# Aman-4-Real/MMTG

Measured on AMD Instinct MI355X. Metric: train tokens/sec, full MMTG config (GPT-2-base-zh decoder, 5x(img+text) 2048-d WenLan embs), higher is better.
Workload: dtype bf16; 1 GPU; Full MMTG train step: S=5 experience steps, T=15+221=236 decoder positions, GPT-2 12L/768/12H V=13317, dropout 0.1 on, MyLoss stage 3 + 0.2*KL, clip 1.0, AdamW; rows_per_gpu=64, global_rows=64, seq_len=236, parallelism=single GPU, no collective

## Files before the change

### include/mmtg_hip.h

```cpp
#ifndef MMTG_HIP_H
#define MMTG_HIP_H

#ifdef __cplusplus
extern "C" {
#endif

#define MMTG_ABI_VERSION 12

#define MMTG_API __attribute__((visibility("default")))

enum { MMTG_OK = 0, MMTG_ERR_BAD_ARG = -1, MMTG_ERR_HIP = -2, MMTG_ERR_UNSUPPORTED = -3 };
enum { MMTG_F32 = 0, MMTG_BF16 = 1 };

enum {
    MMTG_EPI_NONE = 0,
    MMTG_EPI_GELU = 1,
    MMTG_EPI_TANH = 2,
    MMTG_EPI_RESID = 3,
    MMTG_EPI_DGELU = 4,
    MMTG_EPI_DTANH = 5,
    MMTG_EPI_ATOMIC = 6,
    MMTG_EPI_ROWDOT = 7,
    MMTG_EPI_SPLIT = 8,
    MMTG_EPI_TANH_ADD = 9
// ... 128 lines not shown
                      void* dgi, long ld_dgi, void* dgh, float* dh_prev, int B, int H, void* stream);
MMTG_API int mmtg_gru_cell_bwd_fused(int dtype, const void* rows, long ld_rows, const float* carry, const float* part, int splits,
                            const float* save, const void* h_prev, long ld_hp, void* dgi, long ld_dgi, void* dgh,
                            float* dh_prev, int B, int H, void* stream);
#define MMTG_RNN_RELU 0
#define MMTG_RNN_LSTM 1
MMTG_API int mmtg_rnn_cell_fwd(int dtype, int kind, const void* gi, long ld_gi, const void* gh, long ld_gh, const float* c_prev,
                      void* h, long ld_h, float* c, float* save, int B, int H, void* stream);
MMTG_API int mmtg_rnn_cell_bwd(int dtype, int kind, const void* rows, long ld_rows, const float* part, const float* save,
                      const float* c_prev, const void* h, long ld_h, float* dc, int dc_in, void* da, long ld_da,
                      int B, int H, void* stream);
MMTG_API int mmtg_alpha_attn_fwd(int dtype, const void* qkv, const float* prior, void* ctx, float* probs,
                        float* kl, int B, int S, int H, int heads, void* stream);
MMTG_API int mmtg_alpha_attn_bwd(int dtype, const void* qkv, const float* prior, const float* probs,
                        const void* dctx, float dkl, void* dqkv, int B, int S, int H, int heads,
                        void* stream);
MMTG_API int mmtg_beta_fuse_fwd(int dtype, const void* topic, const void* img, const void* txt,
                       const float* att_w, const float* att_b, void* o, float* a,
                       int B, int S, int H, void* stream);
MMTG_API long mmtg_beta_fuse_bwd_ws(int B, int S, int H);
MMTG_API int mmtg_beta_fuse_bwd(int dtype, const void* topic, const void* img, const void* txt,
                       const float* att_w, const float* a, const void* d_o,
                       float* dtopic, void* dimg, void* dtxt, float* datt_w, float* datt_b,
                       int B, int S, int H, float* ws, long ws_floats, void* stream);

MMTG_API int mmtg_prefetch(const void* src, long bytes, int workgroups, void* sink, void* stream);
MMTG_API int mmtg_zero_ranges(float* base, const long* desc, int n, void* stream);

MMTG_API long mmtg_sumsq_ws(long n);
MMTG_API int mmtg_sumsq(const float* x, long n, float* out, float* ws, long ws_floats, void* stream);
MMTG_API int mmtg_adamw(float* p, const float* g, float* m, float* v, void* p_bf16, void* p_lo, long n,
               float lr, float beta1, float beta2, float eps, float wd, int step,
               const float* normsq, float max_norm, float grad_scale, const float* count, void* stream);
MMTG_API int mmtg_cast_f32_to(int dtype, const float* src, void* dst, long n, void* stream);
MMTG_API int mmtg_cast_pad_rows(int dtype, const float* src, long lds_, void* dst, long ldd, int rows, int cols, void* stream);
MMTG_API int mmtg_cast_to_f32(int dtype, const void* src, float* dst, long n, void* stream);
MMTG_API int mmtg_axpy_f32(float* y, const float* x, float a, long n, void* stream);
MMTG_API int mmtg_slab_sum(const float* part, int splits, long stride, float* dst, int accumulate, long n, void* stream);
typedef struct mmtg_wgrad_problem {
    const void* A; long lda;
    const void* B; long ldb;
    float* C; long ldc;
    int M, N;
    long planeA, planeB;
} mmtg_wgrad_problem;
MMTG_API int mmtg_wgrad_group(int config, int n, const mmtg_wgrad_problem* probs, int K, int splits, float* ws, long ws_floats,
                     unsigned* counters, long n_counters, int accumulate, void* stream);
MMTG_API int mmtg_transpose_batch(int dtype, const void* src, void* dst, const long* desc, int n, int max_rows, int max_cols, void* stream);

MMTG_API int mmtg_logits_process_argmax(const float* logits, long ldl, int V, const long long* generated,
                               long ldg, const int* gen_len, float temperature, float rep_penalty,
                               long long* next, int B, void* stream);
MMTG_API int mmtg_logits_process_sample(const float* logits, long ldl, int V, const long long* generated, long ldg,
                               const int* gen_len, float temperature, float rep_penalty, int top_k, float top_p,
                               const float* uniforms, long long* next, float* filtered, int B, void* stream);

MMTG_API int mmtg_decode_embed(int dtype, const void* table, const long long* seq, long ldseq, const void* c, void* x,
                      const int* pos_ptr, const long long* tpw_type, const long long* tpw_mask,
                      long long* type_out, int* keep, long ldkeep, int B, int P, int S, int E, int two_sents,
                      int V, int sent, int max_sent_num, void* stream);
MMTG_API int mmtg_decode_embed_add(int dtype, const void* g, const void* wpe, const void* wte, const long long* type_ids,
                          const int* pos_ptr, void* h, int B, int D, float* stats, void* stream);
MMTG_API int mmtg_decode_gemm(int mode, int M, int N, int K, const void* A, long lda, const void* W, long ldw, void* C, long ldc,
                     const float* bias, const float* colsum, const float* stats_in, int np_in, float eps, int act, int out_f32,
                     const void* resid, long ldr, float* stats_out, int splits, float* ws, long ws_floats, unsigned* counters,
                     long n_counters, const void* emb_pos, const void* emb_type, const long long* type_ids, const int* pos_ptr,
// ... 133 lines not shown
```

### mmtg_amd/csrc/optim.hip

```cpp
#include "common.h"

namespace {

__global__ __launch_bounds__(256) void sumsq_kernel(const float* __restrict__ x, long n, float* __restrict__ out) {
    __shared__ float sh[4];
    float a = 0.f;
    const long n4 = n >> 2;
    for (long i = (long)blockIdx.x * 256 + threadIdx.x; i < n4; i += (long)gridDim.x * 256) {
        f32x4 v = reinterpret_cast<const f32x4*>(x)[i];
        a += v[0] * v[0] + v[1] * v[1] + v[2] * v[2] + v[3] * v[3];
    }
    if (blockIdx.x == 0)
        for (long i = (n4 << 2) + threadIdx.x; i < n; i += 256) a += x[i] * x[i];
    a = wave_sum(a);
    if ((threadIdx.x & 63) == 0) sh[threadIdx.x >> 6] = a;
    __syncthreads();
    if (threadIdx.x == 0) out[blockIdx.x] = sh[0] + sh[1] + sh[2] + sh[3];
}

__global__ __launch_bounds__(256) void sumsq_final_kernel(const float* __restrict__ part, int n, float* __restrict__ out) {
    __shared__ float sh[4];
    float a = 0.f;
    for (int i = threadIdx.x; i < n; i += 256) a += part[i];
    a = wave_sum(a);
// ... 22 lines not shown
    for (long i = (long)blockIdx.x * 256 + threadIdx.x; i < n4; i += (long)gridDim.x * 256) {
        const f32x4 g4 = reinterpret_cast<const f32x4*>(g)[i];
        f32x4 m4 = reinterpret_cast<f32x4*>(m)[i], v4 = reinterpret_cast<f32x4*>(v)[i], p4 = reinterpret_cast<f32x4*>(p)[i];
        bf16x4 c4, l4;
#pragma unroll
        for (int e = 0; e < 4; ++e) {
            const float gi = g4[e] * coef;
            const float mi = b1 * m4[e] + (1.f - b1) * gi;
            const float vi = b2 * v4[e] + (1.f - b2) * gi * gi;
            float pi = p4[e] - step_size * (mi / (sqrtf(vi) + eps));
            if (wd > 0.f) pi -= lr * wd * pi;
            m4[e] = mi; v4[e] = vi; p4[e] = pi;
            c4[e] = (bf16)pi;
            l4[e] = (bf16)(pi - (float)c4[e]);
        }
        reinterpret_cast<f32x4*>(m)[i] = m4;
        reinterpret_cast<f32x4*>(v)[i] = v4;
        reinterpret_cast<f32x4*>(p)[i] = p4;
        if (pc) reinterpret_cast<bf16x4*>(pc)[i] = c4;
        if (pl) reinterpret_cast<bf16x4*>(pl)[i] = l4;
    }
    for (long i = (n4 << 2) + (long)blockIdx.x * 256 + threadIdx.x; i < n; i += (long)gridDim.x * 256) {
        const float gi = g[i] * coef;
        const float mi = b1 * m[i] + (1.f - b1) * gi;
        const float vi = b2 * v[i] + (1.f - b2) * gi * gi;
        float pi = p[i] - step_size * (mi / (sqrtf(vi) + eps));
        if (wd > 0.f) pi -= lr * wd * pi;
        m[i] = mi; v[i] = vi; p[i] = pi;
        if (pc) pc[i] = (bf16)pi;
        if (pl) pl[i] = (bf16)(pi - (float)(bf16)pi);
    }
}

template <typename T>
__global__ __launch_bounds__(256) void cast_from_f32_kernel(const float* __restrict__ src, T* __restrict__ dst, long n) {
    for (long i = (long)blockIdx.x * 256 + threadIdx.x; i < n; i += (long)gridDim.x * 256) dst[i] = (T)src[i];
}
template <typename T>
__global__ __launch_bounds__(256) void cast_to_f32_kernel(const T* __restrict__ src, float* __restrict__ dst, long n) {
    for (long i = (long)blockIdx.x * 256 + threadIdx.x; i < n; i += (long)gridDim.x * 256) dst[i] = (float)src[i];
}
template <typename T>
__global__ __launch_bounds__(256) void cast_pad_rows_kernel(const float* __restrict__ src, long lds_, T* __restrict__ dst,
                                                            long ldd, int cols) {
    const long r = blockIdx.x;
    for (int c = threadIdx.x; c < ldd; c += 256) dst[r * ldd + c] = c < cols ? (T)src[r * lds_ + c] : (T)0.f;
}
__global__ __launch_bounds__(256) void axpy_kernel(float* __restrict__ y, const float* __restrict__ x, float a, long n) {
    for (long i = (long)blockIdx.x * 256 + threadIdx.x; i < n; i += (long)gridDim.x * 256) y[i] += a * x[i];
}

__global__ __launch_bounds__(256) void slab_sum_kernel(const float* __restrict__ part, int splits, long stride,
                                                       float* __restrict__ dst, int accumulate, long n4) {
    typedef float f4 __attribute__((ext_vector_type(4)));
    for (long i = (long)blockIdx.x * 256 + threadIdx.x; i < n4; i += (long)gridDim.x * 256) {
        const f4* src = reinterpret_cast<const f4*>(part) + i;
        f4 acc = accumulate ? reinterpret_cast<const f4*>(dst)[i] : f4{0.f, 0.f, 0.f, 0.f};
        int s = 0;
        for (; s + 4 <= splits; s += 4) {
            const f4 a = src[(s + 0) * (stride / 4)], b = src[(s + 1) * (stride / 4)];
            const f4 c = src[(s + 2) * (stride / 4)], d = src[(s + 3) * (stride / 4)];
            acc += a; acc += b; acc += c; acc += d;
        }
        for (; s < splits; ++s) acc += src[s * (stride / 4)];
        reinterpret_cast<f4*>(dst)[i] = acc;
    }
// ... 68 lines not shown
    MMTG_LAUNCH_CHECK("zero_ranges");
    return MMTG_OK;
}

extern "C" long mmtg_sumsq_ws(long n) { return (long)grid_for(n / 4 + 1); }

extern "C" int mmtg_sumsq(const float* x, long n, float* out, float* ws, long ws_floats, void* stream) {
    MMTG_REQUIRE(x && out && n > 0 && MMTG_ALIGNED16(x), "sumsq: bad args");
    const int g = grid_for(n / 4 + 1);
    MMTG_REQUIRE(ws && ws_floats >= g, "sumsq: workspace of %d floats required (mmtg_sumsq_ws)", g);
    hipStream_t s = (hipStream_t)stream;
    ProfScope prof(MMTG_PROF_OPTIM, s, 2.0 * n, 4.0 * n);
    hipLaunchKernelGGL(sumsq_kernel, dim3(g), dim3(256), 0, s, x, n, ws);
    hipLaunchKernelGGL(sumsq_final_kernel, dim3(1), dim3(256), 0, s, (const float*)ws, g, out);
    MMTG_LAUNCH_CHECK("sumsq");
    return MMTG_OK;
}

extern "C" int mmtg_adamw(float* p, const float* g, float* m, float* v, void* p_bf16, void* p_lo, long n,
                          float lr, float beta1, float beta2, float eps, float wd, int step,
                          const float* normsq, float max_norm, float grad_scale, const float* count, void* stream) {
    MMTG_REQUIRE(p && g && m && v && n > 0 && step >= 1, "adamw: bad args");
    MMTG_REQUIRE(!p_lo || p_bf16, "adamw: the lo plane comes with the hi plane (p_bf16)");
    hipStream_t s = (hipStream_t)stream;
    ProfScope prof(MMTG_PROF_OPTIM, s, 12.0 * n, (28.0 + (p_bf16 ? 2 : 0) + (p_lo ? 2 : 0)) * n);
    const double bc1 = 1.0 - pow((double)beta1, step), bc2 = 1.0 - pow((double)beta2, step);
    const float step_size = (float)((double)lr * sqrt(bc2) / bc1);
    hipLaunchKernelGGL(adamw_kernel, dim3(grid_for(n / 4 + 1)), dim3(256), 0, s, p, g, m, v, (bf16*)p_bf16, (bf16*)p_lo, n, lr, beta1, beta2,
                       eps, wd, step_size, normsq, max_norm, grad_scale, count);
    MMTG_LAUNCH_CHECK("adamw");
    return MMTG_OK;
}

extern "C" int mmtg_cast_f32_to(int dtype, const float* src, void* dst, long n, void* stream) {
    MMTG_REQUIRE(src && dst && n > 0, "cast_f32_to: bad args");
    hipStream_t s = (hipStream_t)stream;
    ProfScope prof(MMTG_PROF_MISC, s, 0, 6.0 * n);
    if (dtype == MMTG_BF16) hipLaunchKernelGGL(cast_from_f32_kernel<bf16>, dim3(grid_for(n)), dim3(256), 0, s, src, (bf16*)dst, n);
    else if (dtype == MMTG_F32) hipLaunchKernelGGL(cast_from_f32_kernel<float>, dim3(grid_for(n)), dim3(256), 0, s, src, (float*)dst, n);
    else MMTG_FAIL(MMTG_ERR_BAD_ARG, "cast_f32_to: bad dtype");
    MMTG_LAUNCH_CHECK("cast_f32_to");
    return MMTG_OK;
}

extern "C" int mmtg_cast_to_f32(int dtype, const void* src, float* dst, long n, void* stream) {
    MMTG_REQUIRE(src && dst && n > 0, "cast_to_f32: bad args");
    hipStream_t s = (hipStream_t)stream;
    ProfScope prof(MMTG_PROF_MISC, s, 0, 6.0 * n);
    if (dtype == MMTG_BF16) hipLaunchKernelGGL(cast_to_f32_kernel<bf16>, dim3(grid_for(n)), dim3(256), 0, s, (const bf16*)src, dst, n);
    else if (dtype == MMTG_F32) hipLaunchKernelGGL(cast_to_f32_kernel<float>, dim3(grid_for(n)), dim3(256), 0, s, (const float*)src, dst, n);
    else MMTG_FAIL(MMTG_ERR_BAD_ARG, "cast_to_f32: bad dtype");
    MMTG_LAUNCH_CHECK("cast_to_f32");
    return MMTG_OK;
}

extern "C" int mmtg_cast_pad_rows(int dtype, const float* src, long lds_, void* dst, long ldd, int rows, int cols, void* stream) {
    MMTG_REQUIRE(src && dst && rows > 0 && cols > 0 && ldd >= cols && lds_ >= cols, "cast_pad_rows: bad args");
    hipStream_t s = (hipStream_t)stream;
    ProfScope prof(MMTG_PROF_MISC, s, 0, 6.0 * rows * cols);
    if (dtype == MMTG_BF16) hipLaunchKernelGGL(cast_pad_rows_kernel<bf16>, dim3(rows), dim3(256), 0, s, src, lds_, (bf16*)dst, ldd, cols);
    else if (dtype == MMTG_F32) hipLaunchKernelGGL(cast_pad_rows_kernel<float>, dim3(rows), dim3(256), 0, s, src, lds_, (float*)dst, ldd, cols);
    else MMTG_FAIL(MMTG_ERR_BAD_ARG, "cast_pad_rows: bad dtype");
    MMTG_LAUNCH_CHECK("cast_pad_rows");
    return MMTG_OK;
}

// ... 36 lines not shown
```

### mmtg_amd/engine.py

```python
from __future__ import annotations

import contextlib
import math

import numpy as np
import torch

from . import hip
from .configs import rnn_param_shapes

ALIGN = 64


class ParamLayout:

    def __init__(self, model_cfgs, gpt2_cfg):
        S = model_cfgs["seq_len"]
        E = model_cfgs["topic"]["input_dim"]
        H = model_cfgs["topic"]["hidden_dim"]
        D = gpt2_cfg["n_embd"]
        V = gpt2_cfg["vocab_size"]
        NP = gpt2_cfg["n_positions"]
        L = gpt2_cfg["n_layer"]
        self.Vpad = (V + 127) // 128 * 128
# ... 119 lines not shown
def _dist_rank():
    import torch.distributed as dist
    return dist.get_rank() if dist.is_available() and dist.is_initialized() else int(_os.environ.get("RANK", "0"))


_NO_OCC4 = bool(_os.environ.get("MMTG_GEMM_NO_OCC4"))
_WG_NUM = float(_os.environ.get("MMTG_WGRAD_NUM", "760"))
_WG_CAP = int(_os.environ.get("MMTG_WGRAD_CAP", "12"))
_NO_FEW_ROWS = bool(_os.environ.get("MMTG_NO_FEW_ROWS"))
_WGRAD_SLAB = not _os.environ.get("MMTG_WGRAD_ATOMIC")
_NO_GATHER = bool(_os.environ.get("MMTG_NO_GATHER"))
_PREFETCH = int(_os.environ.get("MMTG_PREFETCH", "0"))


def _wgrad_splits(M, N, K, occ4=False, slots=512, t_iter=1.1, t_fixed=6.0):
    tiles = ((M + 127) // 128) * ((N + 127) // 128)
    if occ4 and not _NO_OCC4:
        smax = max(1, K // 256)
        s = round(_WG_NUM / tiles) if tiles < 512 else round(2520.0 / tiles)
        return int(max(1, min(smax, s, _WG_CAP)))
    best, best_t = 1, None
    for s in range(1, 33):
        if s > 1 and K // s < 256:
            break
        rounds = -(-tiles * s // slots)
        t = rounds * (K / (64.0 * s) * t_iter + t_fixed) + tiles * s * 65536 / 1.3e6
        if best_t is None or t < best_t * 0.97:
            best, best_t = s, t
    return best


_LAZY_ZERO = _os.environ.get("MMTG_FULL_ZERO_GRAD") is None
_WTE_T = _os.environ.get("MMTG_NO_WTE_T") is None
_P8T = _os.environ.get("MMTG_GEMM_P8T", "0") != "0"
_WGRAD_GROUP = _os.environ.get("MMTG_WGRAD_GROUP", "1") != "0"
_WGRAD_GROUP_SPLITS = int(_os.environ.get("MMTG_WGRAD_GROUP_SPLITS", "0"))
_GELU_GRAD = _os.environ.get("MMTG_GELU_GRAD", "0") != "0"
_DEFER_SUMS = _os.environ.get("MMTG_DEFER_SUMS", "1") != "0"
_WGRAD_TAIL = int(_os.environ.get("MMTG_WGRAD_TAIL", "8"))
_TAIL_FORK_EARLY = _os.environ.get("MMTG_WGRAD_TAIL_FORK", "loop") == "loop"
_LMHEAD_GROUP = _os.environ.get("MMTG_LMHEAD_GROUP", "1") != "0"
_LMHEAD_GROUP_SPLITS = int(_os.environ.get("MMTG_LMHEAD_GROUP_SPLITS", "0"))
_WGRAD_STREAM = _os.environ.get("MMTG_WGRAD_STREAM", "0") != "0"
_ENC_STREAMS = _os.environ.get("MMTG_ENC_STREAMS", "0") != "0"
_HYBRID_ENC_BF16 = _os.environ.get("MMTG_HYBRID_ENC_BF16", "1") != "0"
_X3_WG_CFG = 6 if _os.environ.get("MMTG_WGRAD_X3_COMBINED", "1") != "0" else 2
_WGRAD_GROUP_CFG = int(_os.environ.get("MMTG_WGRAD_GROUP_CFG", "0"))


def _group_splits(tiles, K, slots=1024):
    if _WGRAD_GROUP_SPLITS > 0:
        return _WGRAD_GROUP_SPLITS
    return int(max(1, min(slots // max(1, tiles), K // 1024, 16)))


def _group_splits_x3(tiles, K):
    if _X3_WG_CFG != 6:
        return _group_splits(tiles, K)
    if _WGRAD_GROUP_SPLITS > 0:
        return _WGRAD_GROUP_SPLITS
    s = 512 // max(1, tiles)
    if s == 0:
        s = 2048 // tiles
    return int(max(1, min(s, K // 1024, 16)))


# ... 153 lines not shown
            if off < pos:
                return
            if off > pos:
                comp.append((pos, off - pos))
            pos = off + n
        if pos < self.layout.total:
            comp.append((pos, self.layout.total - pos))
        if not ranges or any(o % 4 or c % 4 for o, c in comp):
            return
        self._ow_desc[key] = (torch.tensor(comp, dtype=torch.int64, device=self.dev), frozenset(ranges))

    def _init_transposed(self):
        self.wt = None
        self.wte_t = None
        self.wt_entries = {}
        if self.dtype == hip.F32 and not self.x3:
            return
        pre, desc, off = "decoder.gpt2.transformer.", [], 0
        for l in range(self.sh.L):
            for nm in ("attn.c_attn", "attn.c_proj", "mlp.c_fc", "mlp.c_proj"):
                key = "%sh.%d.%s.weight" % (pre, l, nm)
                soff, shape, n = self.layout.entries[key]
                assert soff % 8 == 0 and shape[0] % 8 == 0 and shape[1] % 8 == 0
                desc.append((soff, shape[0], shape[1], off))
                self.wt_entries[key] = (off, (shape[1], shape[0]), n)
                off += n
        if self.x3:
            key = "decoder.projector_layer2.weight"
            soff, shape, n = self.layout.entries[key]
            if soff % 8 == 0 and shape[0] % 8 == 0 and shape[1] % 8 == 0:
                desc.append((soff, shape[0], shape[1], off))
                self.wt_entries[key] = (off, (shape[1], shape[0]), n)
                off += n
        self.wt = torch.zeros(*((2, off) if self.x3 else (off,)), device=self.dev, dtype=torch.bfloat16)
        self.wt_total = off
        self.wt_desc = torch.tensor(desc, dtype=torch.int64, device=self.dev)
        self.wt_max = (max(d[1] for d in desc), max(d[2] for d in desc))
        woff = self.layout.pack_range["wte"][0]
        self.wte_t = (torch.zeros(*((2,) if self.x3 else ()), self.sh.D, self.layout.Vpad, device=self.dev, dtype=torch.bfloat16)
                      if (_WTE_T or self.x3) else None)
        self.wte_desc = torch.tensor([(woff, self.layout.Vpad, self.sh.D, 0)], dtype=torch.int64, device=self.dev)

    def Wt(self, key):
        if self.x3:
            raise RuntimeError("Engine.Wt: an x3 engine's transposed copies are (hi | lo) plane pairs -- use Wtx()")
        off, shape, n = self.wt_entries[key]
        return self.wt[off:off + n].view(shape)

    def _refresh_transposed(self):
        if self.wt is not None and self.x3:
            for pl in (0, 1):
                hip.transpose_batch(self.wc2[pl], self.wt[pl], self.wt_desc, self.wt_desc.shape[0], *self.wt_max)
                hip.transpose_batch(self.wc2[pl], self.wte_t[pl], self.wte_desc, 1, self.layout.Vpad, self.sh.D)
        elif self.wt is not None:
            hip.transpose_batch(self.wc, self.wt, self.wt_desc, self.wt_desc.shape[0], *self.wt_max)
            if self.wte_t is not None:
                hip.transpose_batch(self.wc, self.wte_t, self.wte_desc, 1, self.layout.Vpad, self.sh.D)

    def refresh_copies(self):
        if self.copies_fresh:
            return
        if self.x3:
            hip.split_planes(self.master, 1, self.layout.total, hip.Planes(self.wc2, 1, self.layout.total))
            self._refresh_transposed()
            self.copies_fresh = True
        elif self.dtype != hip.F32:
            hip.cast_f32_to(self.master, self.wc, self.layout.total)
            self._refresh_transposed()
            self.copies_fresh = True

    def invalidate_copies(self):
        if self.dtype != hip.F32 or self.x3:
            self.copies_fresh = False

# ... 971 lines not shown
                    last = t == S - 1
                    hip.rnn_cell_bwd(code, dh_all[t:], S * H, None if last else tmp32, save[t] if lstm else None,
                                     rec["c"][t - 1] if lstm and t else None, h_all[t:], S * H, dc, not last, dgi[t:], S * G * H, B, H)
                    if t > 0:
                        hip.gemm(dgi[t:], self.W(r + "weight_hh" + sfx), tmp32, B, H, G * H, transB=False, lda=S * G * H, ldb=H,
                                 out_f32=True)
                hip.colsum(dgi, B * S, G * H, self.G(r + "bias_hh" + sfx))
                drec_tm = None
                if S > 1:
                    drec_tm = self.buf("d_a_tm%d" % G, (S - 1, B, G * H))
                    drec_tm.copy_(dgi.view(B, S, G * H)[:, 1:].transpose(0, 1))
            if S > 1:
                hprev_tm = self.buf("h_prev_tm", (S - 1, B, H))
                hprev_tm.copy_(h_all.view(B, S, H)[:, :S - 1].transpose(0, 1))
                hip.gemm(drec_tm, hprev_tm, self.G(r + "weight_hh" + sfx), G * H, H, (S - 1) * B, transA=True, transB=False,
                         lda=G * H, ldb=H, ldc=H, epi=hip.EPI_ATOMIC, splits=1)
            self._wgrad(rec["inp"], dgi, r + "weight_ih" + sfx, r + "bias_ih" + sfx, B * S, "linear")
            if l > 0:
                dh_all = self.buf("d_hx%d" % (l & 1), (B * S, H))
                hip.gemm(dgi, self.W(r + "weight_ih" + sfx), dh_all, B * S, H, G * H, transB=False, ldb=H)
                if layers[l - 1]["drop"] is not None:
                    hip.dropout_apply(dh_all, dh_all, B * S * H, sh.rnn_pdrop, layers[l - 1]["drop"])

    def grad_norm_sq(self):
        hip.sumsq(self.grad, self.layout.total, self.normsq)
        return self.normsq

    def adamw_step(self, lr, max_norm=1.0, betas=(0.9, 0.999), eps=1e-6, wd=0.0, grad_scale=1.0, clip=True, count=None):
        if self.opt_m is None:
            self.opt_m = torch.zeros_like(self.master)
            self.opt_v = torch.zeros_like(self.master)
        self.step_count += 1
        ns = self.grad_norm_sq() if clip else None
        hip.adamw(self.master, self.grad, self.opt_m, self.opt_v,
                  self.wc2[0] if self.x3 else None if self.dtype == hip.F32 else self.wc,
                  self.layout.total, lr, betas[0], betas[1], eps, wd, self.step_count, ns, max_norm, grad_scale, count=count,
                  p_lo=self.wc2[1] if self.x3 else None)
        self._refresh_transposed()
        self.copies_fresh = True
```

### mmtg_amd/hip.py

```python
from __future__ import annotations

import ctypes as C
import os

import torch

F32, BF16 = 0, 1
ABI_VERSION = 12
EPI_NONE, EPI_GELU, EPI_TANH, EPI_RESID, EPI_DGELU, EPI_DTANH, EPI_ATOMIC, EPI_ROWDOT = range(8)
GEMM_NO_TR, GEMM_REGSTAGE, GEMM_SKINNY, GEMM_NO_SKINNY, GEMM_WIDE, GEMM_NO_WIDE = 1, 2, 4, 8, 16, 32
GEMM_PERSIST, GEMM_NO_PERSIST, GEMM_ROW_ORDER, GEMM_OCC4, GEMM_NO_OCC4, GEMM_COL_BLOCK, GEMM_P256, GEMM_NO_P8, GEMM_P8 = 64, 128, 256, 512, 1024, 2048, 4096, 8192, 16384
GEMM_GELU_GRAD = 32768
GEMM_P8_288 = 65536
GEMM_AUX2_BF16 = 131072
PROF_CATS = ["gemm_bf16", "gemm_f32", "attn_fwd", "attn_bwd", "layernorm", "embed", "loss",
             "optim", "encoder", "decode", "misc"]

_LIB_PATH = os.path.join(os.path.dirname(os.path.abspath(__file__)), "libmmtg_hip.so")
_lib = None

_vp, _i, _l, _f, _u = C.c_void_p, C.c_int, C.c_long, C.c_float, C.c_uint

_SIGS = {
    "mmtg_abi_version": ([], _i),
# ... 12 lines not shown
    "mmtg_layernorm_fwd": ([_i, _vp, _vp, _vp, _vp, _vp, _vp, _i, _i, _f, _vp], _i),
    "mmtg_layernorm_bwd_ws": ([_i, _i], _l),
    "mmtg_layernorm_bwd": ([_i, _vp, _vp, _vp, _vp, _vp, _vp, _vp, _vp, _vp, _i, _i, _vp, _u, _u, _vp, _vp, _l, _vp], _i),
    "mmtg_layernorm_bwd_x3": ([_vp, _vp, _vp, _vp, _vp, _vp, _vp, _vp, _vp, _i, _i, _vp, _l, _u, _u, _vp, _vp, _l, _vp], _i),
    "mmtg_attn_fwd": ([_i, _vp, _vp, _vp, _vp, _i, _i, _i, _i, _u, _u, _vp], _i),
    "mmtg_attn_fwd_x3": ([_vp, _l, _vp, _vp, _vp, _l, _vp, _i, _i, _i, _i, _u, _u, _vp], _i),
    "mmtg_attn_bwd_x3": ([_vp, _l, _vp, _vp, _vp, _l, _vp, _vp, _i, _vp, _l, _vp, _l, _vp, _vp, _l, _i, _i, _i, _i, _u, _u, _vp], _i),
    "mmtg_attn_trace": ([_vp], _i),
    "mmtg_attn_bwd": ([_i, _vp, _vp, _vp, _vp, _vp, _vp, _i, _vp, _vp, _vp, _vp, _i, _i, _i, _i, _u, _u, _i, _vp], _i),
    "mmtg_embed_condition": ([_i, _vp, _vp, _vp, _vp, _vp, _i, _i, _i, _i, _i, _i, _i, _vp], _i),
    "mmtg_segment_sum": ([_i, _vp, _vp, _i, _i, _i, _i, _i, _i, _vp], _i),
    "mmtg_embed_add": ([_i, _vp, _vp, _vp, _vp, _vp, _i, _i, _i, _u, _u, _vp], _i),
    "mmtg_embed_add_bwd": ([_i, _vp, _vp, _vp, _vp, _i, _i, _i, _i, _u, _u, _vp, _l, _vp], _i),
    "mmtg_embed_add_bwd_ws": ([_i, _i, _i], _l),
    "mmtg_dropout_apply": ([_i, _vp, _vp, _l, _i, _u, _u, _vp], _i),
    "mmtg_loss_fwd": ([_i, _vp, _l, _i, _vp, _vp, _vp, _i, _i, _i, _i, _i, _f, _vp, _vp, _vp, _vp, _vp, _vp], _i),
    "mmtg_loss_bwd": ([_i, _i, _vp, _l, _i, _vp, _vp, _vp, _vp, _f, _f, _i, _i, _i, _vp, _l, _i, _vp], _i),
    "mmtg_loss_bwd_x3": ([_vp, _l, _i, _vp, _vp, _vp, _vp, _f, _f, _i, _i, _i, _vp, _l, _l, _i, _vp], _i),
    "mmtg_gru_cell_fwd": ([_i, _vp, _l, _vp, _l, _vp, _l, _vp, _l, _vp, _i, _i, _vp], _i),
    "mmtg_gru_cell_bwd_fused": ([_i, _vp, _l, _vp, _vp, _i, _vp, _vp, _l, _vp, _l, _vp, _vp, _i, _i, _vp], _i),
    "mmtg_rnn_cell_fwd": ([_i, _i, _vp, _l, _vp, _l, _vp, _vp, _l, _vp, _vp, _i, _i, _vp], _i),
    "mmtg_rnn_cell_bwd": ([_i, _i, _vp, _l, _vp, _vp, _vp, _vp, _l, _vp, _i, _vp, _l, _i, _i, _vp], _i),
    "mmtg_gru_cell_bwd": ([_i, _vp, _vp, _vp, _l, _vp, _l, _vp, _vp, _i, _i, _vp], _i),
    "mmtg_alpha_attn_fwd": ([_i, _vp, _vp, _vp, _vp, _vp, _i, _i, _i, _i, _vp], _i),
    "mmtg_alpha_attn_bwd": ([_i, _vp, _vp, _vp, _vp, _f, _vp, _i, _i, _i, _i, _vp], _i),
    "mmtg_beta_fuse_fwd": ([_i, _vp, _vp, _vp, _vp, _vp, _vp, _vp, _i, _i, _i, _vp], _i),
    "mmtg_beta_fuse_bwd": ([_i, _vp, _vp, _vp, _vp, _vp, _vp, _vp, _vp, _vp, _vp, _vp, _i, _i, _i, _vp, _l, _vp], _i),
    "mmtg_beta_fuse_bwd_ws": ([_i, _i, _i], _l),
    "mmtg_prefetch": ([_vp, _l, _i, _vp, _vp], _i),
    "mmtg_zero_ranges": ([_vp, _vp, _i, _vp], _i),
    "mmtg_sumsq": ([_vp, _l, _vp, _vp, _l, _vp], _i),
    "mmtg_sumsq_ws": ([_l], _l),
    "mmtg_adamw": ([_vp, _vp, _vp, _vp, _vp, _vp, _l, _f, _f, _f, _f, _f, _i, _vp, _f, _f, _vp, _vp], _i),
    "mmtg_gemm_x3": ([_i, _i, _i, _vp, _l, _l, _vp, _l, _l, _vp, _l, _vp, _l, _l, _vp, _i, _vp, _l, _vp, _u, _u, _i, _vp], _i),
    "mmtg_split_planes": ([_vp, _l, _i, _i, _vp, _l, _l, _vp], _i),
    "mmtg_layernorm_fwd_x3": ([_vp, _vp, _l, _l, _vp, _vp, _vp, _vp, _i, _i, _f, _vp, _vp], _i),
    "mmtg_cast_f32_to": ([_i, _vp, _vp, _l, _vp], _i),
    "mmtg_cast_pad_rows": ([_i, _vp, _l, _vp, _l, _i, _i, _vp], _i),
    "mmtg_cast_to_f32": ([_i, _vp, _vp, _l, _vp], _i),
    "mmtg_axpy_f32": ([_vp, _vp, _f, _l, _vp], _i),
    "mmtg_slab_sum": ([_vp, _i, _l, _vp, _i, _l, _vp], _i),
    "mmtg_wgrad_group": ([_i, _i, _vp, _i, _i, _vp, _l, _vp, _l, _i, _vp], _i),
    "mmtg_transpose_batch": ([_i, _vp, _vp, _vp, _i, _i, _i, _vp], _i),
    "mmtg_logits_process_argmax": ([_vp, _l, _i, _vp, _l, _vp, _f, _f, _vp, _i, _vp], _i),
    "mmtg_decode_embed": ([_i, _vp, _vp, _l, _vp, _vp, _vp, _vp, _vp, _vp, _vp, _l, _i, _i, _i, _i, _i, _i, _i, _i, _vp], _i),
    "mmtg_decode_embed_add": ([_i, _vp, _vp, _vp, _vp, _vp, _vp, _i, _i, _vp, _vp], _i),
    "mmtg_decode_gemm": ([_i, _i, _i, _i, _vp, _l, _vp, _l, _vp, _l, _vp, _vp, _vp, _i, _f, _i, _i, _vp, _l, _vp, _i, _vp, _l, _vp, _l,
                          _vp, _vp, _vp, _vp, _vp], _i),
    "mmtg_ln_fold_weights": ([_vp, _l, _vp, _vp, _vp, _vp, _vp, _vp, _i, _i, _vp], _i),
    "mmtg_decode_gemm_x3": ([_i, _i, _i, _i, _vp, _l, _l, _vp, _l, _l, _vp, _l, _vp, _l, _l, _vp, _vp, _vp, _i, _f, _i, _vp, _l, _vp, _i, _vp, _l,
                             _vp, _l, _vp, _vp, _vp, _vp, _vp], _i),
    "mmtg_ln_fold_weights_x3": ([_vp, _l, _l, _vp, _vp, _vp, _vp, _l, _l, _vp, _vp, _i, _i, _vp], _i),
    "mmtg_decode_attn_split_x3": ([_vp, _i, _vp, _vp, _vp, _vp, _l, _vp, _vp, _l, _i, _i, _i, _i, _vp], _i),
    "mmtg_decode_embed_x3": ([_vp, _vp, _l, _vp, _vp, _l, _vp, _vp, _vp, _vp, _vp, _l, _i, _i, _i, _i, _i, _i, _i, _i, _vp], _i),
    "mmtg_decode_attn": ([_i, _vp, _vp, _vp, _vp, _l, _vp, _vp, _i, _i, _i, _i, _vp], _i),
    "mmtg_decode_attn_split": ([_i, _vp, _i, _vp, _vp, _vp, _vp, _l, _vp, _vp, _i, _i, _i, _i, _vp], _i),
    "mmtg_logits_process_sample": ([_vp, _l, _i, _vp, _l, _vp, _f, _f, _i, _f, _vp, _vp, _vp, _i, _vp], _i),
    "mmtg_decode_sample": ([_vp, _l, _i, _vp, _l, _vp, _i, _i, _f, _f, _i, _f, _vp, _l, _i, _vp, _vp], _i),
    "mmtg_decode_select": ([_vp, _l, _i, _vp, _l, _vp, _i, _i, _f, _f, _i, _vp, _vp], _i),
    "mmtg_decode_advance": ([_vp, _vp], _i),
    "mmtg_decode_attn_split_rows": ([_i, _vp, _i, _vp, _vp, _vp, _vp, _l, _vp, _l, _vp, _vp, _i, _i, _i, _i, _vp], _i),
    "mmtg_decode_attn_split_x3_rows": ([_vp, _i, _vp, _vp, _vp, _vp, _l, _vp, _l, _vp, _vp, _l, _i, _i, _i, _i, _vp], _i),
    "mmtg_decode_beam_candidates": ([_vp, _l, _i, _vp, _l, _vp, _i, _i, _f, _f, _i, _vp, _vp, _i, _vp], _i),
    "mmtg_decode_beam_merge": ([_vp, _vp, _vp, _vp, _l, _vp, _l, _vp, _l, _vp, _i, _i, _i, _i, _vp, _vp], _i),
    "mmtg_decode_select_fixed": ([_vp, _l, _i, _vp, _l, _vp, _i, _i, _f, _f, _i, _vp, _vp, _vp], _i),
    "mmtg_decode_sample_fixed": ([_vp, _l, _i, _vp, _l, _vp, _i, _i, _f, _f, _i, _f, _vp, _l, _i, _vp, _vp, _vp], _i),
# ... 493 lines not shown
    key = (d_o.device, need, _stream())
    ws = _beta_ws.get(key)
    if ws is None:
        if len(_beta_ws) > 64:
            _beta_ws.clear()
        ws = _beta_ws[key] = torch.empty(need, device=d_o.device, dtype=torch.float32)
    _check(lib().mmtg_beta_fuse_bwd(dt(topic), _p(topic), _p(img), _p(txt), _p(att_w), _p(a), _p(d_o), _p(dtopic),
                                    _p(dimg), _p(dtxt), _p(datt_w), _p(datt_b), B, S, H, _p(ws), ws.numel(), _stream()), "beta_fuse_bwd")


def prefetch(t, sink, workgroups=256, stream=None):
    _check(lib().mmtg_prefetch(_p(t), t.numel() * t.element_size(), int(workgroups), _p(sink),
                               _stream() if stream is None else stream.cuda_stream), "prefetch")


_sumsq_ws = {}


def sumsq(x, n, out):
    need = int(lib().mmtg_sumsq_ws(n))
    key = (x.device, need, _stream())
    ws = _sumsq_ws.get(key)
    if ws is None:
        ws = _sumsq_ws[key] = torch.empty(need, device=x.device, dtype=torch.float32)
    _check(lib().mmtg_sumsq(_p(x), n, _p(out), _p(ws), need, _stream()), "sumsq")


def adamw(p, g, m, v, p_bf16, n, lr, beta1, beta2, eps, wd, step, normsq, max_norm, grad_scale=1.0, count=None, p_lo=None):
    _check(lib().mmtg_adamw(_p(p), _p(g), _p(m), _p(v), _p(p_bf16), _p(p_lo), n, float(lr), float(beta1), float(beta2),
                            float(eps), float(wd), int(step), _p(normsq), float(max_norm), float(grad_scale),
                            _p(count), _stream()), "adamw")


def cast_f32_to(src, dst, n):
    _check(lib().mmtg_cast_f32_to(dt(dst), _p(src), _p(dst), n, _stream()), "cast_f32_to")


def cast_pad_rows(src, lds, dst, ldd, rows, cols):
    _check(lib().mmtg_cast_pad_rows(dt(dst), _p(src), lds, _p(dst), ldd, rows, cols, _stream()), "cast_pad_rows")


def cast_to_f32(src, dst, n):
    _check(lib().mmtg_cast_to_f32(dt(src), _p(src), _p(dst), n, _stream()), "cast_to_f32")


def axpy_f32(y, x, a, n):
    _check(lib().mmtg_axpy_f32(_p(y), _p(x), float(a), n, _stream()), "axpy_f32")


def slab_sum(part, splits, stride, dst, n, accumulate=True):
    _check(lib().mmtg_slab_sum(_p(part), splits, stride, _p(dst), int(accumulate), n, _stream()), "slab_sum")


class WgradProblem(C.Structure):
    _fields_ = [("A", C.c_void_p), ("lda", C.c_long), ("B", C.c_void_p), ("ldb", C.c_long),
                ("C", C.c_void_p), ("ldc", C.c_long), ("M", C.c_int), ("N", C.c_int),
                ("planeA", C.c_long), ("planeB", C.c_long)]


def wgrad_group_sizes(shapes, splits, config=0):
    tb, nw = (256, 8) if config else (128, 4)
    tiles = sum(((M + tb - 1) // tb) * ((N + tb - 1) // tb) for (M, N) in shapes)
    return tiles, tiles * splits * tb * tb, tiles * nw


def wgrad_group(problems, K, splits, ws, counters, accumulate=False, config=0):
# ... 311 lines not shown
```

Before: 1.067 million tokens/s.

## Fuse AdamW update with transposed bf16 weight copy via tiled kernel

Adds a tiled AdamW kernel that updates each weight matrix in 64x64 tiles and also writes the transposed bf16 copy (including the wte transpose) through shared memory in the same pass. Non-matrix parameters are handled by a range kernel. This removes the separate transpose/refresh pass over the bf16 weights after the optimizer step, and copies are marked fresh. It adds descriptor binary search per block and a partially uncoalesced strided transposed write, and it relies on alignment conditions that fall back to the old path if unmet.

```diff
diff --git a/include/mmtg_hip.h b/include/mmtg_hip.h
--- a/include/mmtg_hip.h
+++ b/include/mmtg_hip.h
@@ -184,6 +184,10 @@
 MMTG_API int mmtg_adamw(float* p, const float* g, float* m, float* v, void* p_bf16, void* p_lo, long n,
                float lr, float beta1, float beta2, float eps, float wd, int step,
                const float* normsq, float max_norm, float grad_scale, const float* count, void* stream);
+MMTG_API int mmtg_adamw_tiled(float* p, const float* g, float* m, float* v, void* p_bf16, void* p_bf16_t, const long* tile_desc,
+               int n_mats, long n_tiles, const long* range_desc, int n_ranges, long n,
+               float lr, float beta1, float beta2, float eps, float wd, int step,
+               const float* normsq, float max_norm, float grad_scale, const float* count, void* stream);
 MMTG_API int mmtg_cast_f32_to(int dtype, const float* src, void* dst, long n, void* stream);
 MMTG_API int mmtg_cast_pad_rows(int dtype, const float* src, long lds_, void* dst, long ldd, int rows, int cols, void* stream);
 MMTG_API int mmtg_cast_to_f32(int dtype, const void* src, float* dst, long n, void* stream);
diff --git a/mmtg_amd/csrc/optim.hip b/mmtg_amd/csrc/optim.hip
--- a/mmtg_amd/csrc/optim.hip
+++ b/mmtg_amd/csrc/optim.hip
@@ -78,6 +78,106 @@
     }
 }
 
+#define MMTG_ADAMW_PROLOGUE                                                         \
+    if (count) {                                                                    \
+        const float c = *count;                                                     \
+        if (!(c > 0.f)) return;                                                     \
+        gscale *= 1.0f / c;                                                         \
+    }                                                                               \
+    float coef = gscale;                                                            \
+    if (normsq) {                                                                   \
+        const float nrm = sqrtf(*normsq) * gscale;                                  \
+        coef *= fminf(1.0f, max_norm / (nrm + 1e-6f));                              \
+    }
+#define MMTG_ADAMW_VEC4(g4, m4, v4, p4, c4)                                         \
+    _Pragma("unroll") for (int e = 0; e < 4; ++e) {                                 \
+        const float gi = g4[e] * coef;                                              \
+        const float mi = b1 * m4[e] + (1.f - b1) * gi;                              \
+        const float vi = b2 * v4[e] + (1.f - b2) * gi * gi;                         \
+        float pi = p4[e] - step_size * (mi / (sqrtf(vi) + eps));                    \
+        if (wd > 0.f) pi -= lr * wd * pi;                                           \
+        m4[e] = mi; v4[e] = vi; p4[e] = pi;                                         \
+        c4[e] = (bf16)pi;                                                           \
+    }
+
+constexpr int AT_LDT = 64 + 8;
+__global__ __launch_bounds__(256) void adamw_tile_kernel(float* __restrict__ p, const float* __restrict__ g,
+        float* __restrict__ m, float* __restrict__ v, bf16* __restrict__ pc, bf16* __restrict__ pt, const long* __restrict__ desc,
+        int n_mats, float lr, float b1, float b2, float eps, float wd, float step_size, const float* __restrict__ normsq,
+        float max_norm, float gscale, const float* __restrict__ count) {
+    __shared__ __attribute__((aligned(16))) bf16 tile[64 * AT_LDT];
+    MMTG_ADAMW_PROLOGUE
+    int lo = 0, hi = n_mats - 1;
+    while (lo < hi) {
+        const int mid = (lo + hi + 1) >> 1;
+        if (desc[5 * mid + 4] <= (long)blockIdx.x) lo = mid; else hi = mid - 1;
+    }
+    const long* d = desc + 5 * lo;
+    const long so = d[0], dof = d[3];
+    const int rows = (int)d[1], cols = (int)d[2], t = (int)((long)blockIdx.x - d[4]);
+    const int tc = (cols + 63) >> 6;
+    if (t >= ((rows + 63) >> 6) * tc) return;
+    const int r0 = (t / tc) * 64, c0 = (t % tc) * 64;
+    const int tid = threadIdx.x, ch = tid & 15, rr = tid >> 4;
+    f32x4 g4[4], m4[4], v4[4], p4[4];
+    long at[4];
+    bool ok[4];
+#pragma unroll
+    for (int ps = 0; ps < 4; ++ps) {
+        const int r = r0 + rr + ps * 16, c = c0 + ch * 4;
+        ok[ps] = r < rows && c < cols;
+        at[ps] = so + (ok[ps] ? (long)r * cols + c : (long)r0 * cols + c0);
+        g4[ps] = *reinterpret_cast<const f32x4*>(g + at[ps]);
+        m4[ps] = *reinterpret_cast<const f32x4*>(m + at[ps]);
+        v4[ps] = *reinterpret_cast<const f32x4*>(v + at[ps]);
+        p4[ps] = *reinterpret_cast<const f32x4*>(p + at[ps]);
+    }
+#pragma unroll
+    for (int ps = 0; ps < 4; ++ps) {
+        bf16x4 c4;
+        MMTG_ADAMW_VEC4(g4[ps], m4[ps], v4[ps], p4[ps], c4)
+        if (ok[ps]) {
+            *reinterpret_cast<f32x4*>(m + at[ps]) = m4[ps];
+            *reinterpret_cast<f32x4*>(v + at[ps]) = v4[ps];
+            *reinterpret_cast<f32x4*>(p + at[ps]) = p4[ps];
+            *reinterpret_cast<bf16x4*>(pc + at[ps]) = c4;
+        }
+        *reinterpret_cast<bf16x4*>(tile + (rr + ps * 16) * AT_LDT + ch * 4) = c4;
+    }
+    __syncthreads();
+    const int ch8 = tid & 7, r8 = tid >> 3;
+#pragma unroll
+    for (int ps = 0; ps < 2; ++ps) {
+        const int j = r8 + ps * 32;
+        bf16x8 o;
+#pragma unroll
+        for (int e = 0; e < 8; ++e) o[e] = tile[(ch8 * 8 + e) * AT_LDT + j];
+        if (c0 + j < cols && r0 + ch8 * 8 < rows) *reinterpret_cast<bf16x8*>(pt + dof + (long)(c0 + j) * rows + r0 + ch8 * 8) = o;
+    }
+}
+
+__global__ __launch_bounds__(256) void adamw_ranges_kernel(float* __restrict__ p, const float* __restrict__ g,
+        float* __restrict__ m, float* __restrict__ v, bf16* __restrict__ pc, const long* __restrict__ desc, int n_ranges,
+        float lr, float b1, float b2, float eps, float wd, float step_size, const float* __restrict__ normsq,
+        float max_norm, float gscale, const float* __restrict__ count) {
+    MMTG_ADAMW_PROLOGUE
+    for (int r = 0; r < n_ranges; ++r) {
+        const long off = desc[2 * r], n4 = desc[2 * r + 1] >> 2;
+        for (long i = (long)blockIdx.x * 256 + threadIdx.x; i < n4; i += (long)gridDim.x * 256) {
+            const f32x4 g4 = reinterpret_cast<const f32x4*>(g + off)[i];
+            f32x4 m4 = reinterpret_cast<f32x4*>(m + off)[i], v4 = reinterpret_cast<f32x4*>(v + off)[i], p4 = reinterpret_cast<f32x4*>(p + off)[i];
+            bf16x4 c4;
+            MMTG_ADAMW_VEC4(g4, m4, v4, p4, c4)
+            reinterpret_cast<f32x4*>(m + off)[i] = m4;
+            reinterpret_cast<f32x4*>(v + off)[i] = v4;
+            reinterpret_cast<f32x4*>(p + off)[i] = p4;
+            reinterpret_cast<bf16x4*>(pc + off)[i] = c4;
+        }
+    }
+}
+#undef MMTG_ADAMW_PROLOGUE
+#undef MMTG_ADAMW_VEC4
+
 template <typename T>
 __global__ __launch_bounds__(256) void cast_from_f32_kernel(const float* __restrict__ src, T* __restrict__ dst, long n) {
     for (long i = (long)blockIdx.x * 256 + threadIdx.x; i < n; i += (long)gridDim.x * 256) dst[i] = (T)src[i];
@@ -212,6 +312,28 @@
     return MMTG_OK;
 }
 
+extern "C" int mmtg_adamw_tiled(float* p, const float* g, float* m, float* v, void* p_bf16, void* p_bf16_t, const long* tile_desc,
+                                int n_mats, long n_tiles, const long* range_desc, int n_ranges, long n,
+                                float lr, float beta1, float beta2, float eps, float wd, int step,
+                                const float* normsq, float max_norm, float grad_scale, const float* count, void* stream) {
+    MMTG_REQUIRE(p && g && m && v && p_bf16 && p_bf16_t && tile_desc && n > 0 && step >= 1, "adamw_tiled: bad args");
+    MMTG_REQUIRE(n_mats > 0 && n_tiles >= n_mats && n_tiles < (1L << 31) && n_ranges >= 0 && (range_desc || n_ranges == 0),
+                 "adamw_tiled: bad descriptor counts (%d matrices, %ld tiles, %d ranges)", n_mats, n_tiles, n_ranges);
+    MMTG_REQUIRE(MMTG_ALIGNED16(p) && MMTG_ALIGNED16(g) && MMTG_ALIGNED16(m) && MMTG_ALIGNED16(v) && MMTG_ALIGNED16(p_bf16) && MMTG_ALIGNED16(p_bf16_t),
+                 "adamw_tiled: 16-byte aligned buffers required");
+    hipStream_t s = (hipStream_t)stream;
+    ProfScope prof(MMTG_PROF_OPTIM, s, 12.0 * n, 32.0 * n);
+    const double bc1 = 1.0 - pow((double)beta1, step), bc2 = 1.0 - pow((double)beta2, step);
+    const float step_size = (float)((double)lr * sqrt(bc2) / bc1);
+    hipLaunchKernelGGL(adamw_tile_kernel, dim3((unsigned)n_tiles), dim3(256), 0, s, p, g, m, v, (bf16*)p_bf16, (bf16*)p_bf16_t, tile_desc, n_mats,
+                       lr, beta1, beta2, eps, wd, step_size, normsq, max_norm, grad_scale, count);
+    if (n_ranges > 0)
+        hipLaunchKernelGGL(adamw_ranges_kernel, dim3(2048), dim3(256), 0, s, p, g, m, v, (bf16*)p_bf16, range_desc, n_ranges,
+                           lr, beta1, beta2, eps, wd, step_size, normsq, max_norm, grad_scale, count);
+    MMTG_LAUNCH_CHECK("adamw_tiled");
+    return MMTG_OK;
+}
+
 extern "C" int mmtg_cast_f32_to(int dtype, const float* src, void* dst, long n, void* stream) {
     MMTG_REQUIRE(src && dst && n > 0, "cast_f32_to: bad args");
     hipStream_t s = (hipStream_t)stream;
diff --git a/mmtg_amd/engine.py b/mmtg_amd/engine.py
--- a/mmtg_amd/engine.py
+++ b/mmtg_amd/engine.py
@@ -175,6 +175,7 @@
 
 _LAZY_ZERO = _os.environ.get("MMTG_FULL_ZERO_GRAD") is None
 _WTE_T = _os.environ.get("MMTG_NO_WTE_T") is None
+_ADAMW_TILES = _os.environ.get("MMTG_ADAMW_TILES", "1") != "0"
 _P8T = _os.environ.get("MMTG_GEMM_P8T", "0") != "0"
 _WGRAD_GROUP = _os.environ.get("MMTG_WGRAD_GROUP", "1") != "0"
 _WGRAD_GROUP_SPLITS = int(_os.environ.get("MMTG_WGRAD_GROUP_SPLITS", "0"))
@@ -394,14 +395,31 @@
                 desc.append((soff, shape[0], shape[1], off))
                 self.wt_entries[key] = (off, (shape[1], shape[0]), n)
                 off += n
-        self.wt = torch.zeros(*((2, off) if self.x3 else (off,)), device=self.dev, dtype=torch.bfloat16)
+        tiled = _ADAMW_TILES and _WTE_T and not self.x3
+        tail = self.sh.D * self.layout.Vpad if tiled else 0
+        self.wt = torch.zeros(*((2, off) if self.x3 else (off + tail,)), device=self.dev, dtype=torch.bfloat16)
         self.wt_total = off
         self.wt_desc = torch.tensor(desc, dtype=torch.int64, device=self.dev)
         self.wt_max = (max(d[1] for d in desc), max(d[2] for d in desc))
         woff = self.layout.pack_range["wte"][0]
-        self.wte_t = (torch.zeros(*((2,) if self.x3 else ()), self.sh.D, self.layout.Vpad, device=self.dev, dtype=torch.bfloat16)
+        self.wte_t = (self.wt[off:].view(self.sh.D, self.layout.Vpad) if tiled else
+                      torch.zeros(*((2,) if self.x3 else ()), self.sh.D, self.layout.Vpad, device=self.dev, dtype=torch.bfloat16)
                       if (_WTE_T or self.x3) else None)
         self.wte_desc = torch.tensor([(woff, self.layout.Vpad, self.sh.D, 0)], dtype=torch.int64, device=self.dev)
+        self.adamw_tiles = None
+        if tiled:
+            mats = sorted(desc + [(woff, self.layout.Vpad, self.sh.D, off)])
+            rest, pos = [], 0
+            for soff, rows, cols, _ in mats:
+                if soff > pos:
+                    rest.append((pos, soff - pos))
+                pos = soff + rows * cols
+            if pos < self.layout.total:
+                rest.append((pos, self.layout.total - pos))
+            if all(o % 4 == 0 and c % 4 == 0 for o, c in rest) and woff % 8 == 0 and self.sh.D % 8 == 0:
+                tdesc, ntiles = hip.adamw_tile_desc(mats)
+                self.adamw_tiles = (torch.tensor(tdesc, dtype=torch.int64, device=self.dev), ntiles,
+                                    torch.tensor(rest, dtype=torch.int64, device=self.dev) if rest else None)
 
     def Wt(self, key):
         if self.x3:
@@ -1439,6 +1457,12 @@
             self.opt_v = torch.zeros_like(self.master)
         self.step_count += 1
         ns = self.grad_norm_sq() if clip else None
+        if self.wt is not None and self.adamw_tiles is not None:
+            tdesc, ntiles, rest = self.adamw_tiles
+            hip.adamw_tiled(self.master, self.grad, self.opt_m, self.opt_v, self.wc, self.wt, tdesc, ntiles, rest, self.layout.total,
+                            lr, betas[0], betas[1], eps, wd, self.step_count, ns, max_norm, grad_scale, count=count)
+            self.copies_fresh = True
+            return
         hip.adamw(self.master, self.grad, self.opt_m, self.opt_v,
                   self.wc2[0] if self.x3 else None if self.dtype == hip.F32 else self.wc,
                   self.layout.total, lr, betas[0], betas[1], eps, wd, self.step_count, ns, max_norm, grad_scale, count=count,
diff --git a/mmtg_amd/hip.py b/mmtg_amd/hip.py
--- a/mmtg_amd/hip.py
+++ b/mmtg_amd/hip.py
@@ -68,6 +68,7 @@
     "mmtg_sumsq": ([_vp, _l, _vp, _vp, _l, _vp], _i),
     "mmtg_sumsq_ws": ([_l], _l),
     "mmtg_adamw": ([_vp, _vp, _vp, _vp, _vp, _vp, _l, _f, _f, _f, _f, _f, _i, _vp, _f, _f, _vp, _vp], _i),
+    "mmtg_adamw_tiled": ([_vp, _vp, _vp, _vp, _vp, _vp, _vp, _i, _l, _vp, _i, _l, _f, _f, _f, _f, _f, _i, _vp, _f, _f, _vp, _vp], _i),
     "mmtg_gemm_x3": ([_i, _i, _i, _vp, _l, _l, _vp, _l, _l, _vp, _l, _vp, _l, _l, _vp, _i, _vp, _l, _vp, _u, _u, _i, _vp], _i),
     "mmtg_split_planes": ([_vp, _l, _i, _i, _vp, _l, _l, _vp], _i),
     "mmtg_layernorm_fwd_x3": ([_vp, _vp, _l, _l, _vp, _vp, _vp, _vp, _i, _i, _f, _vp, _vp], _i),
@@ -627,6 +628,22 @@
                             _p(count), _stream()), "adamw")
 
 
+def adamw_tile_desc(mats):
+    desc, tiles = [], 0
+    for soff, rows, cols, doff in mats:
+        desc.append((soff, rows, cols, doff, tiles))
+        tiles += ((rows + 63) // 64) * ((cols + 63) // 64)
+    return desc, tiles
+
+
+def adamw_tiled(p, g, m, v, p_bf16, p_bf16_t, tile_desc, n_tiles, range_desc, n, lr, beta1, beta2, eps, wd, step, normsq, max_norm,
+                grad_scale=1.0, count=None):
+    _check(lib().mmtg_adamw_tiled(_p(p), _p(g), _p(m), _p(v), _p(p_bf16), _p(p_bf16_t), _p(tile_desc), tile_desc.shape[0], int(n_tiles),
+                                  _p(range_desc), 0 if range_desc is None else range_desc.shape[0], n,
+                                  float(lr), float(beta1), float(beta2), float(eps), float(wd), int(step), _p(normsq), float(max_norm),
+                                  float(grad_scale), _p(count), _stream()), "adamw_tiled")
+
+
 def cast_f32_to(src, dst, n):
     _check(lib().mmtg_cast_f32_to(dt(dst), _p(src), _p(dst), n, _stream()), "cast_f32_to")
 
```

Measured after the change: 1.071 million tokens/s, median of 6. Within noise of the previous version (+0.3%).
